# rpl-cmu/bevrender

Measured on AMD Instinct MI355X. Metric: samples/sec fwd+bwd, 6-cam 256x704 BEV-lift+corr, higher is better.
Workload: dtype bf16; 1 GPU; cfg3: 6-cam 256x704 features (64x64x176), 200x200 BEV, C=64 h=2 D=5, L=2 encoder layers (TSA+SCA), T=2 (1 no-grad history frame(s) + 1 fwd+bwd), correlation head with contrastive + lifted-structure losses, AdamW; batch 8 per GPU; backbone/render CNN excluded; global_batch=8, per_gpu_batch=8, parallelism=dp1

## Files before the change

### bevrender_amd/csrc/attn_slab_bwd_q.hip

```cpp
#include "attn_tile.h"
#include "attn_tap.h"

#ifdef BEVR_SPROF
__device__ unsigned long long bevr_prof_slab[48];
extern "C" int bevr_debug_prof_slab(unsigned long long* out, int reset) {
  if (reset) { unsigned long long z[48] = {0}; return (int)hipMemcpyToSymbol(HIP_SYMBOL(bevr_prof_slab), z, sizeof(z)); }
  return (int)hipMemcpyFromSymbol(out, HIP_SYMBOL(bevr_prof_slab), 48 * 8);
}
__device__ __forceinline__ unsigned long long sprof_now() {
  unsigned long long t;
  asm volatile("s_waitcnt vmcnt(0) lgkmcnt(0)\n s_memtime %0\n s_waitcnt lgkmcnt(0)" : "=s"(t) : : "memory");
  return t;
}
#define SPROF(var) const unsigned long long var = sprof_now()
#define SPROF_ADD(i, v) pacc[i] += (v)
#else
#define SPROF(var)
#define SPROF_ADD(i, v)
#endif

namespace {

constexpr int SLAB_W_MAX = 24;
constexpr int SLAB_ROW0 = 10;
constexpr int SLAB_PADR = 8;
constexpr int SLAB_RP = 448;
constexpr int SLAB_CH = 25;
constexpr int SQROWS = 31;
constexpr int SNRB = 7;
constexpr int SNWORK = SNRB;
constexpr int STHREADS = (SNWORK + 1) * 64;
constexpr int SEK = 64;
constexpr int SKROW = 80;
constexpr float SLAB_EPS = 0.02f;

struct SlabKey { int A; float fy; float b; int pad; };

struct SlabCK {
  unsigned wA, wB;
  int cell;
  int row;
};

struct SlabLds {
  static constexpr int K_BYTES = SEK * SKROW;
  static constexpr int OFF_V = K_BYTES;
  static constexpr int OFF_CK = 2 * K_BYTES;
  static constexpr int OFF_CT = OFF_CK + SEK * 16;
  static constexpr int BUF = OFF_CT + 32;
};
enum { SF_DONE = 1, SF_FIRST = 2, SF_LAST = 4 };

__host__ __device__ inline int slab_n_rb(int S) { return (S + SQROWS - 1) / SQROWS; }
__host__ __device__ inline int slab_rows(int S) { return SLAB_ROW0 + S + SLAB_PADR + SQROWS * slab_n_rb(S) + 2; }
__host__ __device__ inline size_t slab_lds_bytes(int S, int sw) {
  return (size_t)(sw + 2) * SLAB_RP * 12 + 2 * SlabLds::BUF + 64;
}
__host__ __device__ inline int slab_width(int S) {
  int sw = SLAB_W_MAX;
  while (sw > 1 && slab_lds_bytes(S, sw) > 160 * 1024) --sw;
  return sw;
}
__host__ __device__ inline int slab_xmin(const bevr_attn_desc& d) { return -(d.Wt / 2 + 2) - 1; }
__host__ __device__ inline int slab_count(const bevr_attn_desc& d, int sw) {
  const float rx = (float)(d.Wt - 1) / (2.0f * (float)(d.S - 1));
  const int xmax = (int)((float)(d.S - 1) * rx) + d.Wt + 3;
  return (xmax - slab_xmin(d) + sw) / sw;
}
__host__ __device__ inline int slab_chunks(int S) { return (S + SLAB_CH - 1) / SLAB_CH; }

struct SlabWs {
  size_t off_beg, off_end, off_items, off_cnt, total;
  int n_slab, n_chunk, sw;
};
__host__ __device__ inline SlabWs slab_ws(const bevr_attn_desc& d) {
  SlabWs w;
  w.sw = slab_width(d.S);
  w.n_slab = slab_count(d, w.sw);
  w.n_chunk = slab_chunks(d.S);
  const size_t pg = (size_t)d.n_prob * d.groups;
  size_t o = pg * d.N * sizeof(SlabKey);
  o = (o + 255) & ~(size_t)255;
  w.off_beg = o;
  o += pg * w.n_slab * d.S * 4;
  w.off_end = o;
  o += pg * w.n_slab * d.S * 4;
  o = (o + 255) & ~(size_t)255;
  w.off_items = o;
  o += (size_t)d.n_prob * d.heads * w.n_slab * w.n_chunk * 16;
  w.off_cnt = o;
  o += 256;
  w.total = o;
  return w;
}

__global__ __launch_bounds__(256) void slab_keys_kernel(bevr_attn_desc d, const float* __restrict__ key_a,
                                                        const float* __restrict__ key_b, const int* __restrict__ order,
                                                        SlabKey* __restrict__ out) {
  const size_t t = (size_t)blockIdx.x * 256 + threadIdx.x;
  const size_t total = (size_t)d.n_prob * d.groups * d.N;
  if (t >= total) return;
  const int pg = (int)(t / d.N);
  const int n = order[t];
  float a = key_a[(size_t)pg * d.Np + n], b = key_b[(size_t)pg * d.Np + n];
  const float aL = -(float)(d.Sp + 1), aU = (float)(d.Ht + 1);
  const float half = (float)(d.Wt / 2);
  const float bL = -(half + 2.0f), bU = (float)(d.Wt + 1);
  a = fminf(fmaxf(a, aL), aU);
  b = fminf(fmaxf(b, bL), bU);
  const float af = floorf(a);
  SlabKey k;
  k.A = (int)af;
  k.fy = a - af;
  k.b = b;
  k.pad = 0;
  out[t] = k;
}

__device__ __forceinline__ int slab_lower_bound(const SlabKey* __restrict__ keys, int N, float thr) {
  int lo = 0, hi = N;
  while (lo < hi) {
    const int mid = (lo + hi) >> 1;
    if (keys[mid].b < thr) lo = mid + 1; else hi = mid;
  }
  return lo;
}

__global__ __launch_bounds__(256) void slab_ranges_kernel(bevr_attn_desc d, const SlabKey* __restrict__ keys,
                                                          int* __restrict__ kbeg, int* __restrict__ kend,
                                                          int4* __restrict__ items, int* __restrict__ cnt, int n_slab,
                                                          int n_chunk, int sw) {
  const int t = blockIdx.x * 256 + threadIdx.x;
  const int n_pg = d.n_prob * d.groups;
  if (t >= n_pg * n_slab * n_chunk) return;
  const int chunk = t % n_chunk, slab = (t / n_chunk) % n_slab, pg = t / (n_chunk * n_slab);
  const SlabKey* kp = keys + (size_t)pg * d.N;
  const float rx = (float)(d.Wt - 1) / (2.0f * (float)(d.S - 1));
  const int x0 = slab_xmin(d) + slab * sw;
  int work = 0;
  const int j1 = min(d.S, (chunk + 1) * SLAB_CH);
  for (int j = chunk * SLAB_CH; j < j1; ++j) {
    const float jrx = (float)j * rx;
    const int b0 = slab_lower_bound(kp, d.N, (float)x0 - jrx - SLAB_EPS);
    const int b1 = slab_lower_bound(kp, d.N, (float)(x0 + sw) - jrx + SLAB_EPS);
    kbeg[((size_t)pg * n_slab + slab) * d.S + j] = b0;
    kend[((size_t)pg * n_slab + slab) * d.S + j] = b1;
    work += b1 - b0;
  }
  if (work > 0) {
    const int hpg = d.heads / d.groups;
    const int prob = pg / d.groups, grp = pg % d.groups;
    const int at = atomicAdd(cnt, hpg);
    for (int h = 0; h < hpg; ++h) items[at + h] = make_int4(prob * d.heads + grp * hpg + h, slab, chunk, work);
  }
}

__device__ __forceinline__ float slab_lane_below(float x) {
  return __builtin_bit_cast(float, __builtin_amdgcn_update_dpp(0, __builtin_bit_cast(int, x), 0x138, 0xf, 0xf, true));
}
__device__ __forceinline__ unsigned long long slab_from_int(int v) {
  return ((unsigned long long)(unsigned)(v >> 31) << 32) | (unsigned)v;
}
__device__ __forceinline__ float slab_to_float(unsigned long long v) {
  const int lo = (int)(unsigned)v, hi = (int)(unsigned)(v >> 32);
  if (hi == (lo >> 31)) return (float)lo;
  return (float)(long long)v;
}
__device__ __forceinline__ int half_max_i(int v) {
#pragma unroll
  for (int s = 16; s > 0; s >>= 1) v = max(v, __shfl_xor(v, s));
  return v;
}

#define SLAB_BARRIER() __syncthreads()

template <int PREC>
__global__ __launch_bounds__(STHREADS, 1) void attn_slab_bwd_q_kernel(
    bevr_attn_desc d, const char* __restrict__ Q, const char* __restrict__ Ks, const char* __restrict__ Vs,
    const SlabKey* __restrict__ skeys, const int* __restrict__ kbeg, const int* __restrict__ kend,
    const int4* __restrict__ items, int* __restrict__ cnt, const char* __restrict__ table_pair,
    const char* __restrict__ dO, const float* __restrict__ LSE, const float* __restrict__ delta,
    const float* __restrict__ grad_scale, float* __restrict__ dQ, float* __restrict__ dtable, int n_slab, int sw, int R) {
  typedef SlabLds L;
  extern __shared__ __attribute__((aligned(256))) char lds[];
  constexpr int RP = SLAB_RP;
  const int ncell = (sw + 2) * RP;
  unsigned* vals = reinterpret_cast<unsigned*>(lds);
  unsigned long long* cells = reinterpret_cast<unsigned long long*>(lds + (size_t)ncell * 4);
  char* stage = reinterpret_cast<char*>(cells) + (size_t)ncell * 8;
  int* item_slot = reinterpret_cast<int*>(stage + 2 * L::BUF);

  const int tid = threadIdx.x, wave = tid >> 6, lane = tid & 63, lq = lane & 31, hi = lane >> 5;
  const bool producer = wave == SNWORK;
  const int rb = wave;
  const int n_rb = slab_n_rb(d.S);
  const int Mp = d.S * d.Sp;
  const int Hq = d.Hp + 1;
  const float rx = (float)(d.Wt - 1) / (2.0f * (float)(d.S - 1));
  const int n_items = cnt[0];
  const int hpg = d.heads / d.groups;

  const float gscale = grad_scale[0], ginv = grad_scale[1] * BEVR_LN2;
  const float kp16 = PREC == BEVR_PREC_F16 ? grad_scale[2] : 0.f, c2_16 = PREC == BEVR_PREC_F16 ? grad_scale[3] : 1.f;
  const float cfix = PREC == BEVR_PREC_F16 ? grad_scale[0] * grad_scale[4] : 1.f;
  const float dq_scale = PREC == BEVR_PREC_F16 ? grad_scale[4] * BEVR_LN2 : ginv;
#ifdef BEVR_SPROF
  unsigned long long pacc[16] = {0, 0, 0, 0, 0, 0, 0, 0, 0, 0, 0, 0, 0, 0, 0, 0};
#endif

  for (;;) {
    SLAB_BARRIER();
    if (tid == 0) item_slot[0] = atomicAdd(cnt + 1, 1);
    SLAB_BARRIER();
    const int it = __builtin_amdgcn_readfirstlane(item_slot[0]);
    if (it >= n_items) break;
    const int4 item = items[it];
    const int ph = __builtin_amdgcn_readfirstlane(item.x), slab = __builtin_amdgcn_readfirstlane(item.y),
              chunk = __builtin_amdgcn_readfirstlane(item.z);
    const int prob = ph / d.heads, hd = ph % d.heads;
    const int pg = prob * d.groups + hd / hpg;
    const int qb = prob / d.q_div;
    const int x0 = slab_xmin(d) + slab * sw;
    const int j0 = chunk * SLAB_CH, j1 = min(d.S, j0 + SLAB_CH);
    const char* tbl = table_pair + (size_t)hd * d.Wp * d.Hp * 8;
    float* dtb = dtable + (size_t)hd * d.Wp * Hq;
    SPROF(ti0);

    for (int u = tid; u < (sw + 1) * RP; u += STHREADS) {
      const int c = u / RP, w = u - c * RP;
      const int xc = x0 + c + d.x_off;
      const int yr = w - SLAB_ROW0 + d.y_off;
      f32x2 v = {0.f, 0.f};
      if (w < R && yr >= 0 && yr < d.Hp && xc >= 0 && xc < d.Wp)
        v = *reinterpret_cast<const f32x2*>(tbl + ((size_t)xc * d.Hp + yr) * 8);
      vals[RP + u] = Half<PREC>::pack2(v[0], v[1]);
      cells[RP + u] = 0ull;
    }
    for (int u = tid; u < RP; u += STHREADS) {
      vals[u] = Half<PREC>::pack2(Half<PREC>::NEG_BIG, Half<PREC>::NEG_BIG);
      cells[u] = 0ull;
    }
    SLAB_BARRIER();
    SPROF(ti1);
    SPROF_ADD(12, ti1 - ti0);
    SPROF_ADD(15, 1);

    if (producer) {
      __builtin_amdgcn_s_setprio(3);
      const SlabKey* kp = skeys + (size_t)pg * d.N;
      const char* Kh = Ks + (size_t)ph * d.N * 64;
      const char* Vh = Vs + (size_t)ph * d.N * 64;
      const size_t rbase = ((size_t)pg * n_slab + slab) * d.S;
      const int my_beg = j0 + lane < j1 ? kbeg[rbase + j0 + lane] : 0;
      const int my_end = j0 + lane < j1 ? kend[rbase + j0 + lane] : 0;
      int lc = 0, lk = 0, lend = 0;
      auto seek = [&]() {
        while (lc < j1 - j0) {
          const int b = __builtin_amdgcn_readlane(my_beg, lc), e = __builtin_amdgcn_readlane(my_end, lc);
          if (b < e) { lk = b; lend = e; return; }
          ++lc;
        }
      };
      seek();
      u32x4 kv[8];
      SlabKey sk;
      int cur_c = -1, cur_k = 0, cur_end = 0;
      bool have = false;
      auto issue = [&]() {
        have = lc < j1 - j0;
        if (!have) return;
        cur_c = lc; cur_k = lk; cur_end = lend;
        const int kmax = d.N - 1;
#pragma unroll
        for (int q = 0; q < 4; ++q) {
          const int cid = lane + 64 * q;
          const int key = min(cur_k + (cid >> 2), kmax);
          kv[q] = *reinterpret_cast<const u32x4*>(Kh + (size_t)key * 64 + (cid & 3) * 16);
          kv[4 + q] = *reinterpret_cast<const u32x4*>(Vh + (size_t)key * 64 + (cid & 3) * 16);
        }
        sk = kp[min(cur_k + lane, kmax)];
        lk += SEK;
        if (lk >= lend) { ++lc; seek(); }
      };
      issue();
      int e = 0;
      int prev_c = -1;
      while (have) {
        char* bb = stage + (e & 1) * L::BUF;
        const int c = cur_c, k0 = cur_k, kend_c = cur_end;
        const int j = j0 + c;
        const float jrx = (float)j * rx;
        const bool last = !(lc < j1 - j0) || lc != c;
        const bool first = c != prev_c;
        prev_c = c;
        SPROF(tp0);
        const SlabKey sk_e = sk;
        u32x4 kv_e[8];
#pragma unroll
        for (int q = 0; q < 8; ++q) kv_e[q] = kv[q];
        SPROF(tp1);
        SPROF_ADD(0, tp1 - tp0);
        issue();
        {
          const float tx = jrx + sk_e.b;
          const float xf = floorf(tx);
          const int X = (int)xf;
          const bool live = (k0 + lane < kend_c) && X >= x0 && X < x0 + sw;
          const float fx = tx - xf, fy = sk_e.fy;
          SlabCK ck;
          if (live) {
            ck.wA = Half<PREC>::pack2((1.0f - fx) * (1.0f - fy), (1.0f - fx) * fy);
            ck.wB = Half<PREC>::pack2(fx * (1.0f - fy), fx * fy);
            ck.row = sk_e.A + SLAB_ROW0;
            ck.cell = ((X - x0 + 1) * RP + ck.row) * 4;
          } else {
            ck.wA = Half<PREC>::pack2(1.f, 0.f);
            ck.wB = 0u;
            ck.row = 0;
            ck.cell = 0;
          }
          *reinterpret_cast<SlabCK*>(bb + L::OFF_CK + lane * 16) = ck;
          const bool far = live && (sk_e.A + SLAB_ROW0 < 0 || sk_e.A > d.S - 1 + SLAB_PADR);
          const unsigned long long lm = __ballot(live), fm = __ballot(far);
          const unsigned hb = ((unsigned)lm != 0u ? 1u : 0u) | ((unsigned)(lm >> 32) != 0u ? 2u : 0u) |
                              ((unsigned)fm != 0u ? 4u : 0u) | ((unsigned)(fm >> 32) != 0u ? 8u : 0u);
          const int jn = (last && have) ? j0 + cur_c + 1 : 0;
          if (lane == 0)
            *reinterpret_cast<u32x4*>(bb + L::OFF_CT) =
                u32x4{(unsigned)((first ? SF_FIRST : 0) | (last ? SF_LAST : 0)) | (hb << 8), (unsigned)j | ((unsigned)jn << 16), 0u, 0u};
        }
#pragma unroll
        for (int q = 0; q < 4; ++q) {
          const int cid = lane + 64 * q;
          *reinterpret_cast<u32x4*>(bb + (cid >> 2) * SKROW + (cid & 3) * 16) = kv_e[q];
          *reinterpret_cast<u32x4*>(bb + L::OFF_V + (cid >> 2) * SKROW + (cid & 3) * 16) = kv_e[4 + q];
        }
        ++e;
        SPROF(tp2);
        SPROF_ADD(1, tp2 - tp1);
        SLAB_BARRIER();
        SPROF(tp3);
        SPROF_ADD(2, tp3 - tp2);
        SPROF_ADD(3, 1);
      }
      if (lane == 0) *reinterpret_cast<u32x4*>(stage + (e & 1) * L::BUF + L::OFF_CT) = u32x4{(unsigned)SF_DONE, 0u, 0u, 0u};
      SLAB_BARRIER();
      __builtin_amdgcn_s_setprio(0);
    } else {
      const bool active = rb < n_rb;
      if (wave >= 4) __builtin_amdgcn_s_setprio(1);
      const int i0 = rb * SQROWS;
      const int qrow = i0 + lq;
      const bool live = lq < SQROWS && qrow < d.S;
      const int rowoff4 = (i0 + lq) * 4;
      const char* Qh = Q + ((size_t)(qb * d.heads + hd) * Mp) * 64;
      const char* dOh = dO + ((size_t)ph * Mp) * 64;
      const unsigned cells_off = (unsigned)(reinterpret_cast<char*>(cells) - lds);
      Frag<PREC> qf, dof;
      float nl = 0.f, nd = 0.f, lse_r = 0.f, dlt_r = 0.f;
      int jcur = -1, jpend = -1;
      f32x16 dq;
#pragma unroll
      for (int r = 0; r < 16; ++r) dq[r] = 0.f;

      auto issue_column = [&](int j) {
        const size_t mq = (size_t)j * d.Sp + min(qrow, d.S - 1);
        qf.load(Qh + mq * 64, hi);
        dof.load(dOh + mq * 64, hi);
        lse_r = LSE[(size_t)ph * Mp + mq];
        dlt_r = delta[(size_t)ph * Mp + mq];
        jpend = j;
      };
      auto finish_column = [&]() {
        float dlt = dlt_r;
        if (!live) {
          dof.v[0] = bf16x8{0, 0, 0, 0, 0, 0, 0, 0};
          dof.v[1] = bf16x8{0, 0, 0, 0, 0, 0, 0, 0};
          dlt = 0.f;
        }
        if constexpr (PREC != BEVR_PREC_F16) dlt *= gscale;
        if constexpr (PREC == BEVR_PREC_BF16) {
#pragma unroll
          for (int h = 0; h < 2; ++h) {
            u32x4 w = __builtin_bit_cast(u32x4, dof.v[h]);
#pragma unroll
            for (int k = 0; k < 4; ++k)
              w[k] = pack_bf16x2(__builtin_bit_cast(float, w[k] << 16) * gscale,
                                 __builtin_bit_cast(float, w[k] & 0xffff0000u) * gscale);
            dof.v[h] = __builtin_bit_cast(bf16x8, w);
          }
        }
        nl = kp16 - lse_r;
        nd = -dlt;
        jcur = jpend;
      };
      auto flush_dq = [&]() {
        float* base = dQ + ((size_t)ph * Mp + (size_t)jcur * d.Sp + i0) * 32 + lq;
#pragma unroll
        for (int r = 0; r < 16; ++r) {
          const int qr = crow(r, hi);
          if (qr < SQROWS && i0 + qr < d.S) atomicAdd(base + (size_t)qr * 32, dq_scale * dq[r]);
          dq[r] = 0.f;
        }
      };

      auto process = [&](const char* bb, int jn, auto clamp_tag) {
        constexpr bool CLAMP = decltype(clamp_tag)::value;
        const SlabCK* pk0 = reinterpret_cast<const SlabCK*>(bb + L::OFF_CK);
        f32x16 s[2], dp[2];
        {
          float a = nl, b = nd;
          asm volatile("" : "+v"(a), "+v"(b));
#pragma unroll
          for (int h = 0; h < 2; ++h)
#pragma unroll
            for (int r = 0; r < 16; ++r) { s[h][r] = a; dp[h][r] = b; }
        }
#pragma unroll
        for (int h = 0; h < 2; ++h) {
          Frag<PREC> kf, vkf;
          kf.load(bb + (h * 32 + lq) * SKROW, hi);
          s[h] = mma_frag(kf, qf, s[h]);
          vkf.load(bb + L::OFF_V + (h * 32 + lq) * SKROW, hi);
          dp[h] = mma_frag(vkf, dof, dp[h]);
        }
        if (jn >= 0) issue_column(jn);
        __builtin_amdgcn_sched_barrier(0);
        SPROF(tq0);
        auto offset = [&](const SlabCK& e) -> int {
          if constexpr (CLAMP) return (e.cell - 4 * e.row) + 4 * max(0, min(e.row + (rowoff4 >> 2), R - 1));
          else return e.cell + rowoff4;
        };
        auto read_tap = [&](int off, unsigned& a, unsigned& b) {
          a = *reinterpret_cast<const unsigned*>(lds + off);
          b = *reinterpret_cast<const unsigned*>(lds + off + RP * 4);
        };
        auto dq_product = [&](int h) {
          Frag<PREC> ktf;
          const int i16 = lane & 15, chalf = (lane >> 4) & 1;
          const char* p = bb + (h * 32 + 4 * hi + (i16 >> 2)) * SKROW + chalf * 32 + 8 * (i16 & 3);
          ktf.v[0] = lds_tr8(p, 8 * SKROW);
          ktf.v[1] = lds_tr8(p + 16 * SKROW, 8 * SKROW);
#pragma unroll
          for (int ks = 0; ks < 2; ++ks) {
            u32x4 w;
#pragma unroll
            for (int k = 0; k < 4; ++k) w[k] = Half<PREC>::pack2(s[h][8 * ks + 2 * k], s[h][8 * ks + 2 * k + 1]);
            dq = Half<PREC>::mfma(__builtin_bit_cast(bf16x8, w), ktf.v[ks], dq);
          }
        };
#pragma unroll
        for (int h = 0; h < 2; ++h) {
          const SlabCK* pk = pk0 + h * 32;
          SlabCK e0[2], e1[2];
          int o0[2];
          unsigned ta[2], tb[2];
#pragma unroll
          for (int c = 0; c < 2; ++c) {
            e0[c] = pk[crow(8 * c, hi)];
            e1[c] = pk[crow(8 * c + 1, hi)];
            o0[c] = offset(e0[c]);
            read_tap(o0[c], ta[c], tb[c]);
          }
#pragma unroll
          for (int r = 0; r < 8; ++r) {
            unsigned na[2], nb[2];
            SlabCK e2[2];
            int o1[2];
#pragma unroll
            for (int c = 0; c < 2; ++c) {
              na[c] = ta[c]; nb[c] = tb[c]; e2[c] = e1[c]; o1[c] = o0[c];
              if (r + 1 < 8) { o1[c] = offset(e1[c]); read_tap(o1[c], na[c], nb[c]); }
              if (r + 2 < 8) e2[c] = pk[crow(8 * c + r + 2, hi)];
            }
            int iA[2], iB[2];
#pragma unroll
            for (int c = 0; c < 2; ++c) {
              const int row = 8 * c + r;
              float sv = Half<PREC>::dot2(ta[c], e0[c].wA, s[h][row]);
              sv = Half<PREC>::dot2(tb[c], e0[c].wB, sv);
              float ds = fast_exp2(sv) * dp[h][row];
              if constexpr (PREC == BEVR_PREC_F16) ds *= c2_16;
              s[h][row] = ds;
              const float gb_ = slab_lane_below(ds);
              if constexpr (PREC == BEVR_PREC_BF16) {
                const unsigned pr = pack_bf16x2(ds, gb_);
                asm("v_dot2_f32_bf16 %0, %2, %3, 0\n\t"
                    "v_dot2_f32_bf16 %1, %2, %4, 0\n\t"
                    "s_nop 2\n\t"
                    "v_cvt_rpi_i32_f32 %0, %0\n\t"
                    "v_cvt_rpi_i32_f32 %1, %1"
                    : "=&v"(iA[c]), "=&v"(iB[c])
                    : "v"(pr), "v"(e0[c].wA), "v"(e0[c].wB));
              } else {
                const unsigned pr = Half<PREC>::pack2(ds, gb_);
                asm("v_dot2_f32_f16 %0, %2, %3, 0\n\t"
                    "v_dot2_f32_f16 %1, %2, %4, 0\n\t"
                    "s_nop 2\n\t"
                    "v_mul_f32 %0, %0, %5\n\t"
                    "v_mul_f32 %1, %1, %5\n\t"
                    "v_cvt_rpi_i32_f32 %0, %0\n\t"
                    "v_cvt_rpi_i32_f32 %1, %1"
                    : "=&v"(iA[c]), "=&v"(iB[c])
                    : "v"(pr), "v"(e0[c].wA), "v"(e0[c].wB), "v"(cfix));
              }
            }
#pragma unroll
            for (int c = 0; c < 2; ++c) {
              unsigned long long* gp = reinterpret_cast<unsigned long long*>(lds + cells_off + 2 * o0[c]);
              atomicAdd(gp, slab_from_int(iA[c]));
              atomicAdd(gp + RP, slab_from_int(iB[c]));
              e0[c] = e1[c]; e1[c] = e2[c]; ta[c] = na[c]; tb[c] = nb[c]; o0[c] = o1[c];
            }
          }
          dq_product(h);
          __builtin_amdgcn_sched_barrier(0);
        }
        SPROF(tq1);
        SPROF_ADD(4, tq1 - tq0);
      };

      int e = 0;
      for (;;) {
        SPROF(tw0);
        SLAB_BARRIER();
        SPROF(tw1);
        SPROF_ADD(0, tw1 - tw0);
        const char* bb = stage + (e & 1) * L::BUF;
        const u32x4 ct = *reinterpret_cast<const u32x4*>(bb + L::OFF_CT);
        const unsigned flags = (unsigned)__builtin_amdgcn_readfirstlane((int)ct[0]);
        const unsigned jword = (unsigned)__builtin_amdgcn_readfirstlane((int)ct[1]);
        if (flags & SF_DONE) break;
        if (active) {
          const int j = (int)(jword & 0xffffu);
          if (flags & SF_FIRST) {
            if (jpend != j) issue_column(j);
            finish_column();
          }
          const unsigned hb = flags >> 8;
          if (hb & 3u) {
            const int jn = (flags & SF_LAST) ? (int)(jword >> 16) - 1 : -1;
            if (hb & 12u) process(bb, jn, std::true_type{});
            else process(bb, jn, std::false_type{});
          }
          if (flags & SF_LAST) flush_dq();
        }
        SPROF(tw2);
        SPROF_ADD(1, tw2 - tw1);
        SPROF_ADD(2, (flags >> 8) & 1u);
        SPROF_ADD(3, 1);
        ++e;
      }
    }

    SLAB_BARRIER();
    SPROF(tf0);
    for (int u = tid; u < (sw + 1) * RP; u += STHREADS) {
      const int c = u / RP, w = u - c * RP;
      const unsigned long long v = w < R ? cells[RP + u] : 0ull;
      if (v != 0ull) {
        const int xc = x0 + c + d.x_off, yr = w - SLAB_ROW0 + d.y_off;
        if (xc >= 0 && xc < d.Wp && yr >= 0 && yr < Hq) atomicAdd(dtb + (size_t)xc * Hq + yr, slab_to_float(v) * ginv);
      }
    }
    SPROF(tf1);
    SPROF_ADD(13, tf1 - tf0);
  }
#ifdef BEVR_SPROF
  if (lane == 0 && (wave == 0 || wave == SNWORK - 1 || producer)) {
    const int base = producer ? 32 : (wave ? 16 : 0);
    for (int i = 0; i < 16; ++i) atomicAdd(&bevr_prof_slab[base + i], pacc[i]);
  }
#endif
}

template <int PREC>
int launch(const bevr_attn_desc& d, const void* Q, const void* Ks, const void* Vs, const void* ws, const float* table_pair,
           const void* dO, const float* LSE, const float* delta, const float* grad_scale, float* dQ, float* dtable,
           hipStream_t st) {
  const SlabWs w = slab_ws(d);
  const char* base = static_cast<const char*>(ws);
  int* cnt = reinterpret_cast<int*>(const_cast<char*>(base) + w.off_cnt);
  hipError_t e = hipMemsetAsync(cnt + 1, 0, 4, st);
  if (e != hipSuccess) return (int)e;
  static int n_cu = 0;
  if (n_cu == 0) {
    int dev = 0;
    hipDeviceProp_t prop;
    if (hipGetDevice(&dev) != hipSuccess || hipGetDeviceProperties(&prop, dev) != hipSuccess) return BEVR_E_SHAPE;
    n_cu = prop.multiProcessorCount;
  }
  const int R = slab_rows(d.S);
  const size_t lds = slab_lds_bytes(d.S, w.sw);
  static bool attr_set[4] = {false, false, false, false};
  if (!attr_set[PREC]) {
    e = hipFuncSetAttribute(reinterpret_cast<const void*>(&attn_slab_bwd_q_kernel<PREC>),
                            hipFuncAttributeMaxDynamicSharedMemorySize, 160 * 1024);
    if (e != hipSuccess) return (int)e;
    attr_set[PREC] = true;
  }
  hipLaunchKernelGGL((attn_slab_bwd_q_kernel<PREC>), dim3(n_cu), dim3(STHREADS), lds, st, d, (const char*)Q,
                     (const char*)Ks, (const char*)Vs, reinterpret_cast<const SlabKey*>(base),
                     reinterpret_cast<const int*>(base + w.off_beg), reinterpret_cast<const int*>(base + w.off_end),
                     reinterpret_cast<const int4*>(base + w.off_items), cnt, (const char*)table_pair, (const char*)dO,
                     LSE, delta, grad_scale, dQ, dtable, w.n_slab, w.sw, R);
  return (int)hipGetLastError();
}

bool slab_shape_ok(const bevr_attn_desc& d) {
  return is16(d.precision) && slab_n_rb(d.S) <= SNRB && slab_rows(d.S) <= SLAB_RP && SLAB_CH <= 64 &&
         slab_lds_bytes(d.S, slab_width(d.S)) <= 160 * 1024;
}

}

extern "C" size_t bevr_attn_slab_ws_bytes(const bevr_attn_desc* d) {
  if (bevr_check_desc(d) || !slab_shape_ok(*d)) return 0;
  return slab_ws(*d).total;
}

extern "C" int bevr_attn_slab_prep(const bevr_attn_desc* d, const float* key_a, const float* key_b, const int* order,
                                   void* slab_ws_, void* stream) {
  int rc = bevr_check_desc(d);
  if (rc) return rc;
  if (!key_a || !key_b || !order || !slab_ws_) return BEVR_E_NULL;
  if (!is16(d->precision)) return BEVR_E_PRECISION;
  if (!slab_shape_ok(*d)) return BEVR_E_SHAPE;
  if (!bevr_aligned16(slab_ws_)) return BEVR_E_ALIGN;
  const SlabWs w = slab_ws(*d);
  char* base = static_cast<char*>(slab_ws_);
  hipStream_t st = (hipStream_t)stream;
  hipError_t e = hipMemsetAsync(base + w.off_cnt, 0, 256, st);
  if (e != hipSuccess) return (int)e;
  const size_t nk = (size_t)d->n_prob * d->groups * d->N;
  hipLaunchKernelGGL(slab_keys_kernel, dim3((unsigned)((nk + 255) / 256)), dim3(256), 0, st, *d, key_a, key_b, order,
                     reinterpret_cast<SlabKey*>(base));
  const int nt = d->n_prob * d->groups * w.n_slab * w.n_chunk;
  hipLaunchKernelGGL(slab_ranges_kernel, dim3((nt + 255) / 256), dim3(256), 0, st, *d,
                     reinterpret_cast<const SlabKey*>(base), reinterpret_cast<int*>(base + w.off_beg),
                     reinterpret_cast<int*>(base + w.off_end), reinterpret_cast<int4*>(base + w.off_items),
                     reinterpret_cast<int*>(base + w.off_cnt), w.n_slab, w.n_chunk, w.sw);
  return (int)hipGetLastError();
}

extern "C" int bevr_attn_slab_bwd_q(const bevr_attn_desc* d, const void* Q, const void* Ks, const void* Vs,
                                    const void* slab_ws_, const float* table_pair, const void* dO, const float* LSE,
                                    const float* delta, const float* grad_scale, float* dQ, float* dtable, void* stream) {
  int rc = bevr_check_desc(d);
  if (rc) return rc;
  if (!Q || !Ks || !Vs || !slab_ws_ || !table_pair || !dO || !LSE || !delta || !grad_scale || !dQ || !dtable)
    return BEVR_E_NULL;
  if (!is16(d->precision)) return BEVR_E_PRECISION;
  if (!slab_shape_ok(*d)) return BEVR_E_SHAPE;
  if (!bevr_aligned16(Q) || !bevr_aligned16(Ks) || !bevr_aligned16(Vs) || !bevr_aligned16(dO) || !bevr_aligned16(dQ) ||
      !bevr_aligned16(table_pair) || !bevr_aligned16(slab_ws_))
    return BEVR_E_ALIGN;
  hipStream_t st = (hipStream_t)stream;
  if (d->precision == BEVR_PREC_BF16)
    return launch<BEVR_PREC_BF16>(*d, Q, Ks, Vs, slab_ws_, table_pair, dO, LSE, delta, grad_scale, dQ, dtable, st);
  return launch<BEVR_PREC_F16>(*d, Q, Ks, Vs, slab_ws_, table_pair, dO, LSE, delta, grad_scale, dQ, dtable, st);
}
```

Measured before the change: 5.687 samples/s.

## Batch two key tiles per barrier with a 4-slot ring and XOR-swizzled K/V rows

The producer wave now stages two 64-key K/V tiles into a four-slot LDS ring before each workgroup barrier, and the consumer waves process both tiles per barrier. This halves the number of block-wide syncs on the slab dQ backward. The K/V row pitch drops from 80 to 64 bytes, with an XOR swizzle on the 16-byte chunks so the MFMA fragment and transposed loads avoid bank conflicts. The ring adds LDS, which can shrink the slab width, and the host launcher's static caches become per-device atomics.

```diff
diff --git a/bevrender_amd/csrc/attn_slab_bwd_q.hip b/bevrender_amd/csrc/attn_slab_bwd_q.hip
--- a/bevrender_amd/csrc/attn_slab_bwd_q.hip
+++ b/bevrender_amd/csrc/attn_slab_bwd_q.hip
@@ -1,5 +1,6 @@
 #include "attn_tile.h"
 #include "attn_tap.h"
+#include <atomic>
 
 #ifdef BEVR_SPROF
 __device__ unsigned long long bevr_prof_slab[48];
@@ -31,7 +32,9 @@
 constexpr int SNWORK = SNRB;
 constexpr int STHREADS = (SNWORK + 1) * 64;
 constexpr int SEK = 64;
-constexpr int SKROW = 80;
+constexpr int SEPB = 2;
+constexpr int SRING = 2 * SEPB;
+constexpr int SKROW = 64;
 constexpr float SLAB_EPS = 0.02f;
 
 struct SlabKey { int A; float fy; float b; int pad; };
@@ -49,12 +52,13 @@
   static constexpr int OFF_CT = OFF_CK + SEK * 16;
   static constexpr int BUF = OFF_CT + 32;
 };
+__device__ __forceinline__ int slab_krow(int n, int c) { return n * SKROW + ((c ^ ((n >> 2) & 3)) << 4); }
 enum { SF_DONE = 1, SF_FIRST = 2, SF_LAST = 4 };
 
 __host__ __device__ inline int slab_n_rb(int S) { return (S + SQROWS - 1) / SQROWS; }
 __host__ __device__ inline int slab_rows(int S) { return SLAB_ROW0 + S + SLAB_PADR + SQROWS * slab_n_rb(S) + 2; }
 __host__ __device__ inline size_t slab_lds_bytes(int S, int sw) {
-  return (size_t)(sw + 2) * SLAB_RP * 12 + 2 * SlabLds::BUF + 64;
+  return (size_t)(sw + 2) * SLAB_RP * 12 + (size_t)SRING * SlabLds::BUF + 64;
 }
 __host__ __device__ inline int slab_width(int S) {
   int sw = SLAB_W_MAX;
@@ -188,7 +192,7 @@
   unsigned* vals = reinterpret_cast<unsigned*>(lds);
   unsigned long long* cells = reinterpret_cast<unsigned long long*>(lds + (size_t)ncell * 4);
   char* stage = reinterpret_cast<char*>(cells) + (size_t)ncell * 8;
-  int* item_slot = reinterpret_cast<int*>(stage + 2 * L::BUF);
+  int* item_slot = reinterpret_cast<int*>(stage + SRING * L::BUF);
 
   const int tid = threadIdx.x, wave = tid >> 6, lane = tid & 63, lq = lane & 31, hi = lane >> 5;
   const bool producer = wave == SNWORK;
@@ -283,10 +287,23 @@
         if (lk >= lend) { ++lc; seek(); }
       };
       issue();
-      int e = 0;
+      int sp = 0;
       int prev_c = -1;
-      while (have) {
-        char* bb = stage + (e & 1) * L::BUF;
+      for (bool done = false; !done; sp ^= 1) {
+       SPROF(ts0);
+#pragma nounroll
+       for (int i = 0; i < SEPB; ++i) {
+        const int slot = sp * SEPB + i;
+#ifdef BEVR_DEBUG
+        if (slot < 0 || slot >= SRING || stage + (size_t)(slot + 1) * L::BUF > reinterpret_cast<char*>(item_slot))
+          __builtin_trap();
+#endif
+        char* bb = stage + slot * L::BUF;
+        if (!have) {
+          if (lane == 0) *reinterpret_cast<u32x4*>(bb + L::OFF_CT) = u32x4{(unsigned)SF_DONE, 0u, 0u, 0u};
+          done = true;
+          break;
+        }
         const int c = cur_c, k0 = cur_k, kend_c = cur_end;
         const int j = j0 + c;
         const float jrx = (float)j * rx;
@@ -332,19 +349,20 @@
 #pragma unroll
         for (int q = 0; q < 4; ++q) {
           const int cid = lane + 64 * q;
-          *reinterpret_cast<u32x4*>(bb + (cid >> 2) * SKROW + (cid & 3) * 16) = kv_e[q];
-          *reinterpret_cast<u32x4*>(bb + L::OFF_V + (cid >> 2) * SKROW + (cid & 3) * 16) = kv_e[4 + q];
-        }
-        ++e;
+          *reinterpret_cast<u32x4*>(bb + slab_krow(cid >> 2, cid & 3)) = kv_e[q];
+          *reinterpret_cast<u32x4*>(bb + L::OFF_V + slab_krow(cid >> 2, cid & 3)) = kv_e[4 + q];
+        }
         SPROF(tp2);
         SPROF_ADD(1, tp2 - tp1);
-        SLAB_BARRIER();
-        SPROF(tp3);
-        SPROF_ADD(2, tp3 - tp2);
         SPROF_ADD(3, 1);
+       }
+       SPROF(tp3);
+       SLAB_BARRIER();
+       SPROF(tp4);
+       SPROF_ADD(2, tp4 - tp3);
+       SPROF_ADD(5, tp3 - ts0);
+       SPROF_ADD(6, 1);
       }
-      if (lane == 0) *reinterpret_cast<u32x4*>(stage + (e & 1) * L::BUF + L::OFF_CT) = u32x4{(unsigned)SF_DONE, 0u, 0u, 0u};
-      SLAB_BARRIER();
       __builtin_amdgcn_s_setprio(0);
     } else {
       const bool active = rb < n_rb;
@@ -419,9 +437,11 @@
 #pragma unroll
         for (int h = 0; h < 2; ++h) {
           Frag<PREC> kf, vkf;
-          kf.load(bb + (h * 32 + lq) * SKROW, hi);
+          kf.v[0] = *reinterpret_cast<const bf16x8*>(bb + slab_krow(h * 32 + lq, hi));
+          kf.v[1] = *reinterpret_cast<const bf16x8*>(bb + slab_krow(h * 32 + lq, 2 + hi));
           s[h] = mma_frag(kf, qf, s[h]);
-          vkf.load(bb + L::OFF_V + (h * 32 + lq) * SKROW, hi);
+          vkf.v[0] = *reinterpret_cast<const bf16x8*>(bb + L::OFF_V + slab_krow(h * 32 + lq, hi));
+          vkf.v[1] = *reinterpret_cast<const bf16x8*>(bb + L::OFF_V + slab_krow(h * 32 + lq, 2 + hi));
           dp[h] = mma_frag(vkf, dof, dp[h]);
         }
         if (jn >= 0) issue_column(jn);
@@ -438,9 +458,11 @@
         auto dq_product = [&](int h) {
           Frag<PREC> ktf;
           const int i16 = lane & 15, chalf = (lane >> 4) & 1;
-          const char* p = bb + (h * 32 + 4 * hi + (i16 >> 2)) * SKROW + chalf * 32 + 8 * (i16 & 3);
-          ktf.v[0] = lds_tr8(p, 8 * SKROW);
-          ktf.v[1] = lds_tr8(p + 16 * SKROW, 8 * SKROW);
+          const int n = h * 32 + 4 * hi + (i16 >> 2), ch = 2 * chalf + ((i16 >> 1) & 1), sub = 8 * (i16 & 1);
+          const char* p = bb + slab_krow(n, ch) + sub;
+          const int off2 = slab_krow(n + 8, ch) - slab_krow(n, ch);
+          ktf.v[0] = lds_tr8(p, off2);
+          ktf.v[1] = lds_tr8(p + 16 * SKROW, off2);
 #pragma unroll
           for (int ks = 0; ks < 2; ++ks) {
             u32x4 w;
@@ -520,17 +542,26 @@
         SPROF_ADD(4, tq1 - tq0);
       };
 
-      int e = 0;
-      for (;;) {
-        SPROF(tw0);
-        SLAB_BARRIER();
-        SPROF(tw1);
-        SPROF_ADD(0, tw1 - tw0);
-        const char* bb = stage + (e & 1) * L::BUF;
+      int sp = 0;
+      for (bool done = false; !done; sp ^= 1) {
+       SPROF(tw0);
+       SLAB_BARRIER();
+       SPROF(tw1);
+       SPROF_ADD(0, tw1 - tw0);
+       SPROF_ADD(6, 1);
+#pragma nounroll
+       for (int i = 0; i < SEPB; ++i) {
+        const int slot = sp * SEPB + i;
+#ifdef BEVR_DEBUG
+        if (slot / SEPB != sp || slot >= SRING || stage + (size_t)(slot + 1) * L::BUF > reinterpret_cast<char*>(item_slot))
+          __builtin_trap();
+#endif
+        SPROF(te0);
+        const char* bb = stage + slot * L::BUF;
         const u32x4 ct = *reinterpret_cast<const u32x4*>(bb + L::OFF_CT);
         const unsigned flags = (unsigned)__builtin_amdgcn_readfirstlane((int)ct[0]);
         const unsigned jword = (unsigned)__builtin_amdgcn_readfirstlane((int)ct[1]);
-        if (flags & SF_DONE) break;
+        if (flags & SF_DONE) { done = true; break; }
         if (active) {
           const int j = (int)(jword & 0xffffu);
           if (flags & SF_FIRST) {
@@ -545,11 +576,11 @@
           }
           if (flags & SF_LAST) flush_dq();
         }
-        SPROF(tw2);
-        SPROF_ADD(1, tw2 - tw1);
+        SPROF(te1);
+        SPROF_ADD(1, te1 - te0);
         SPROF_ADD(2, (flags >> 8) & 1u);
         SPROF_ADD(3, 1);
-        ++e;
+       }
       }
     }
 
@@ -583,21 +614,25 @@
   int* cnt = reinterpret_cast<int*>(const_cast<char*>(base) + w.off_cnt);
   hipError_t e = hipMemsetAsync(cnt + 1, 0, 4, st);
   if (e != hipSuccess) return (int)e;
-  static int n_cu = 0;
+  constexpr int MAX_DEV = 64;
+  static std::atomic<int> n_cu_of[MAX_DEV];
+  static std::atomic<bool> attr_set[MAX_DEV];
+  int dev = 0;
+  if (hipGetDevice(&dev) != hipSuccess || dev < 0 || dev >= MAX_DEV) return BEVR_E_SHAPE;
+  int n_cu = n_cu_of[dev].load(std::memory_order_relaxed);
   if (n_cu == 0) {
-    int dev = 0;
-    hipDeviceProp_t prop;
-    if (hipGetDevice(&dev) != hipSuccess || hipGetDeviceProperties(&prop, dev) != hipSuccess) return BEVR_E_SHAPE;
-    n_cu = prop.multiProcessorCount;
+    if (hipDeviceGetAttribute(&n_cu, hipDeviceAttributeMultiprocessorCount, dev) != hipSuccess || n_cu <= 0)
+      return BEVR_E_SHAPE;
+    n_cu_of[dev].store(n_cu, std::memory_order_relaxed);
   }
   const int R = slab_rows(d.S);
   const size_t lds = slab_lds_bytes(d.S, w.sw);
-  static bool attr_set[4] = {false, false, false, false};
-  if (!attr_set[PREC]) {
+  if (lds > 160 * 1024) return BEVR_E_SHAPE;
+  if (!attr_set[dev].load(std::memory_order_acquire)) {
     e = hipFuncSetAttribute(reinterpret_cast<const void*>(&attn_slab_bwd_q_kernel<PREC>),
                             hipFuncAttributeMaxDynamicSharedMemorySize, 160 * 1024);
     if (e != hipSuccess) return (int)e;
-    attr_set[PREC] = true;
+    attr_set[dev].store(true, std::memory_order_release);
   }
   hipLaunchKernelGGL((attn_slab_bwd_q_kernel<PREC>), dim3(n_cu), dim3(STHREADS), lds, st, d, (const char*)Q,
                      (const char*)Ks, (const char*)Vs, reinterpret_cast<const SlabKey*>(base),
```

Result: no change. 5.727 samples/s, median of 6 (+0.7%).
